# teamtomo/torch-motion-correction

Measured on AMD Instinct MI355X. Metric: frames/sec motion-corrected, 40×4k×4k fp32 stack, 1/2/4/8 MI355X, higher is better.
Workload: dtype f32; 1 GPU; 40-frame 4096x4096 fp32 movie, global rigid shift estimate+correct (estimate_global_motion -> correct_motion, frames + sum out), 1 stack per GPU per step, consecutive steps overlapped on two HIP streams; b_factor=500

## Files before the change

torch_motion_correction_amd/csrc/mc_wave_fft.h:

```cpp
#pragma once

#ifdef __HIPCC__
#include "mc_common.h"
#define MC_HD __host__ __device__ __forceinline__
#else
#include <math.h>
#include <stdint.h>
struct cfloat {
  float x, y;
};
#define MC_HD static inline
#endif

typedef float wf2 __attribute__((ext_vector_type(2)));

#define WF_N 2048
#define WF_SLAB 1024

#ifdef __HIPCC__
__device__ __forceinline__ void wf_sync() {
  __builtin_amdgcn_fence(__ATOMIC_RELEASE, "wavefront");
  __builtin_amdgcn_wave_barrier();
  __builtin_amdgcn_fence(__ATOMIC_ACQUIRE, "wavefront");
}
#endif

MC_HD wf2 wf_make(float re, float im) { return wf2{re, im}; }
MC_HD wf2 wf_from(cfloat c) { return wf2{c.x, c.y}; }
MC_HD cfloat wf_to(wf2 v) { return cfloat{v.x, v.y}; }

MC_HD wf2 wf_add_mi(wf2 a, wf2 b) {
#if defined(__HIP_DEVICE_COMPILE__)
  wf2 r;
  asm("v_pk_add_f32 %0, %1, %2 op_sel:[0,1] op_sel_hi:[1,0] neg_hi:[0,1]" : "=v"(r) : "v"(a), "v"(b));
  return r;
#else
  return wf2{a.x + b.y, a.y - b.x};
#endif
}
MC_HD wf2 wf_sub_mi(wf2 a, wf2 b) {
#if defined(__HIP_DEVICE_COMPILE__)
  wf2 r;
  asm("v_pk_add_f32 %0, %1, %2 op_sel:[0,1] op_sel_hi:[1,0] neg_lo:[0,1]" : "=v"(r) : "v"(a), "v"(b));
  return r;
#else
  return wf2{a.x - b.y, a.y + b.x};
#endif
}
MC_HD wf2 wf_cmul(wf2 a, wf2 w) {
#if defined(__HIP_DEVICE_COMPILE__)
  wf2 t, r;
  asm("v_pk_mul_f32 %0, %1, %2 op_sel_hi:[0,1]" : "=v"(t) : "v"(a), "v"(w));
  asm("v_pk_fma_f32 %0, %1, %2, %3 op_sel:[1,1,0] op_sel_hi:[1,0,1] neg_lo:[0,1,0]"
      : "=v"(r)
      : "v"(a), "v"(w), "v"(t));
  return r;
#else
  return wf2{a.x * w.x - a.y * w.y, a.x * w.y + a.y * w.x};
#endif
}
MC_HD wf2 wf_fma_c(wf2 a, wf2 b, float cr, float ci) {
  const wf2 c = {cr, ci}, cs = {-ci, cr};
  return __builtin_elementwise_fma(b.yy, cs, __builtin_elementwise_fma(b.xx, c, a));
}
MC_HD wf2 wf_cmulc(wf2 a, float cr, float ci) {
  const wf2 c = {cr, ci}, cs = {-ci, cr};
  return __builtin_elementwise_fma(a.yy, cs, a.xx * c);
}

MC_HD void wf_bfly4(wf2& a0, wf2& a1, wf2& a2, wf2& a3) {
  const wf2 t0 = a0 + a2, t1 = a0 - a2;
  const wf2 t2 = a1 + a3, d = a1 - a3;
  a0 = t0 + t2;
  a2 = t0 - t2;
  a1 = wf_add_mi(t1, d);
  a3 = wf_sub_mi(t1, d);
}

MC_HD void wf_dft16(wf2 (&a)[16]) {
  const float C1 = 0.92387953251128673848f, S1 = 0.38268343236508978178f;
  const float H = 0.70710678118654752440f;
#pragma unroll
  for (int j = 0; j < 4; ++j) wf_bfly4(a[j], a[j + 4], a[j + 8], a[j + 12]);
  a[1 + 4] = wf_cmulc(a[1 + 4], C1, -S1);
  a[1 + 8] = wf_cmulc(a[1 + 8], H, -H);
  a[1 + 12] = wf_cmulc(a[1 + 12], S1, -C1);
  a[2 + 4] = wf_cmulc(a[2 + 4], H, -H);
  a[2 + 12] = wf_cmulc(a[2 + 12], -H, -H);
  a[3 + 4] = wf_cmulc(a[3 + 4], S1, -C1);
  a[3 + 8] = wf_cmulc(a[3 + 8], -H, -H);
  a[3 + 12] = wf_cmulc(a[3 + 12], -C1, S1);
#pragma unroll
  for (int p = 0; p < 4; ++p) {
    wf2 &b0 = a[4 * p], &b1 = a[4 * p + 1], &b2 = a[4 * p + 2], &b3 = a[4 * p + 3];
    if (p == 2) {
      const wf2 t0 = wf_add_mi(b0, b2), t1 = wf_sub_mi(b0, b2);
      const wf2 t2 = b1 + b3, d = b1 - b3;
      b0 = t0 + t2;
      b2 = t0 - t2;
      b1 = wf_add_mi(t1, d);
      b3 = wf_sub_mi(t1, d);
    } else {
      wf_bfly4(b0, b1, b2, b3);
    }
  }
#pragma unroll
  for (int p = 0; p < 4; ++p)
#pragma unroll
    for (int r = p + 1; r < 4; ++r) {
      const wf2 s = a[4 * p + r];
      a[4 * p + r] = a[4 * r + p];
      a[4 * r + p] = s;
    }
}

MC_HD void wf_dft16_lo2(wf2 (&a)[16]) {
  const float C1 = 0.92387953251128673848f, S1 = 0.38268343236508978178f;
  const float H = 0.70710678118654752440f;
  const wf2 x0 = a[0], x1 = a[1], x2 = a[14], x3 = a[15];
  a[0] = x0; a[4] = x0; a[8] = x0; a[12] = x0;
  a[1] = x1;
  a[1 + 4] = wf_cmulc(x1, C1, -S1);
  a[1 + 8] = wf_cmulc(x1, H, -H);
  a[1 + 12] = wf_cmulc(x1, S1, -C1);
  a[2] = x2;
  a[2 + 4] = wf_cmulc(x2, H, H);
  a[2 + 8] = -x2;
  a[2 + 12] = wf_cmulc(x2, -H, H);
  a[3] = x3;
  a[3 + 4] = wf_cmulc(x3, C1, S1);
  a[3 + 8] = wf_cmulc(x3, H, H);
  a[3 + 12] = wf_cmulc(x3, S1, C1);
#pragma unroll
  for (int p = 0; p < 4; ++p) {
    wf2 &b0 = a[4 * p], &b1 = a[4 * p + 1], &b2 = a[4 * p + 2], &b3 = a[4 * p + 3];
    if (p == 2) {
      const wf2 t0 = wf_add_mi(b0, b2), t1 = wf_sub_mi(b0, b2);
      const wf2 t2 = b1 + b3, d = b1 - b3;
      b0 = t0 + t2;
      b2 = t0 - t2;
      b1 = wf_add_mi(t1, d);
      b3 = wf_sub_mi(t1, d);
    } else {
      wf_bfly4(b0, b1, b2, b3);
    }
  }
#pragma unroll
  for (int p = 0; p < 4; ++p)
#pragma unroll
    for (int r = p + 1; r < 4; ++r) {
      const wf2 s = a[4 * p + r];
      a[4 * p + r] = a[4 * r + p];
      a[4 * r + p] = s;
    }
}

template <int KEEP>
MC_HD void wf_dft8_pruned(const wf2 (&e)[4], const wf2 (&o)[4], wf2 (&z)[8]) {
  const float H = 0.70710678118654752440f;
  wf2 e0 = e[0], e1 = e[1], e2 = e[2], e3 = e[3];
  wf2 o0 = o[0], o1 = o[1], o2 = o[2], o3 = o[3];
  wf_bfly4(e0, e1, e2, e3);
  wf_bfly4(o0, o1, o2, o3);
  z[0] = e0 + o0;
  z[7] = wf_fma_c(e3, o3, H, H);
  if (KEEP >= 2) {
    z[1] = wf_fma_c(e1, o1, H, -H);
    z[6] = wf_sub_mi(e2, o2);
  }
  if (KEEP >= 4) {
    z[2] = wf_add_mi(e2, o2);
    z[3] = wf_fma_c(e3, o3, -H, -H);
    z[4] = e0 - o0;
    z[5] = wf_fma_c(e1, o1, -H, H);
  }
}

struct WfLane {
  int x1w_base, x1w_mask;
  int x1r[4];
  int x2w;
  int x2r[4];
  int kbin[4];
  int self;
};

MC_HD WfLane wf_lane(int t) {
  WfLane L;
  {
    const int n2 = t >> 2, h1 = (t >> 1) & 1, h0 = t & 1;
    L.x1w_base = (n2 * 2 + h1) * 32 + h0 * 16;
    L.x1w_mask = (n2 & 3) | (h1 << 2) | (h0 << 3);
  }
  {
    const int k1 = t & 15, g2 = t >> 4, h1 = g2 >> 1, h0 = g2 & 1;
    const int lanepart = h1 * 32 + h0 * 16, lo = k1 ^ ((h1 << 2) | (h0 << 3));
    for (int v = 0; v < 4; ++v) L.x1r[v] = lanepart + (lo ^ v);
    L.x2w = g2 * 256 + k1;
  }
  L.kbin[0] = t;
  L.kbin[1] = t == 0 ? 128 : 256 - t;
  L.kbin[2] = 64 + t;
  L.kbin[3] = 192 - t;
  for (int s = 0; s < 4; ++s) L.x2r[s] = L.kbin[s];
  L.self = t == 0;
  return L;
}

MC_HD wf2 wf_unpack(wf2 zk, wf2 zmr, wf2 wk) {
  const wf2 zm = {zmr.x, -zmr.y};
  const wf2 sm = zk + zm, d = zk - zm;
  const wf2 wd = wf_cmul(d, wk);
  return wf_add_mi(sm, wd) * 0.5f;
}

template <int KEEP>
MC_HD void wf_unpack_lane(const wf2 (&z)[4][8], const wf2 (&wk)[4], bool self, wf2 (&X)[4][KEEP]) {
  const float C1 = 0.92387953251128673848f, S1 = 0.38268343236508978178f;
#pragma unroll
  for (int k3 = 0; k3 < KEEP; ++k3) {
    const wf2 m_a0 = self ? z[0][(8 - k3) & 7] : z[1][7 - k3];
    const wf2 m_a1 = self ? z[1][7 - k3] : z[0][7 - k3];
    wf2 w[4] = {wk[0], wk[1], wk[2], wk[3]};
    if (k3 == 1) {
#pragma unroll
      for (int s = 0; s < 4; ++s) w[s] = wf_cmulc(w[s], C1, -S1);
    }
    X[0][k3] = wf_unpack(z[0][k3], m_a0, w[0]);
    X[1][k3] = wf_unpack(z[1][k3], m_a1, w[1]);
    X[2][k3] = wf_unpack(z[2][k3], z[3][7 - k3], w[2]);
    X[3][k3] = wf_unpack(z[3][k3], z[2][7 - k3], w[3]);
  }
}

#define WF5_N 512
#define WF5_SLAB 512

MC_HD void wf_dft8(wf2 (&a)[8]) {
  const float H = 0.70710678118654752440f;
  wf2 e0 = a[0], e1 = a[2], e2 = a[4], e3 = a[6];
  wf2 o0 = a[1], o1 = a[3], o2 = a[5], o3 = a[7];
  wf_bfly4(e0, e1, e2, e3);
  wf_bfly4(o0, o1, o2, o3);
  a[0] = e0 + o0;
  a[4] = e0 - o0;
  a[1] = wf_fma_c(e1, o1, H, -H);
  a[5] = wf_fma_c(e1, o1, -H, H);
  a[2] = wf_add_mi(e2, o2);
  a[6] = wf_sub_mi(e2, o2);
  a[3] = wf_fma_c(e3, o3, -H, -H);
  a[7] = wf_fma_c(e3, o3, H, H);
}

MC_HD int wf5_x1(int k1, int n2, int n3) { return ((n2 * 8 + (k1 ^ n2)) * 8) + (n3 ^ (4 * (k1 >> 2))); }
MC_HD int wf5_x2(int k2, int n3, int k1) { return ((n3 * 8 + (k2 ^ n3)) * 8) + k1; }

#define WF10_N 1024
MC_HD int wf10_x1(int k1, int q) { return k1 * 64 + (q ^ ((2 * k1) & 31)); }
MC_HD int wf10_x2(int k1, int k2, int n3) { return n3 * 128 + k2 * 16 + k1; }

MC_HD void wf_twiddle8(wf2 (&a)[8], wf2 w1) {
  const wf2 w2 = wf_cmul(w1, w1), w3 = wf_cmul(w2, w1), w4 = wf_cmul(w2, w2);
  a[1] = wf_cmul(a[1], w1);
  a[2] = wf_cmul(a[2], w2);
  a[3] = wf_cmul(a[3], w3);
  a[4] = wf_cmul(a[4], w4);
  a[5] = wf_cmul(a[5], wf_cmul(w4, w1));
  a[6] = wf_cmul(a[6], wf_cmul(w4, w2));
  a[7] = wf_cmul(a[7], wf_cmul(w4, w3));
}
MC_HD void wf_twiddle16(wf2 (&a)[16], wf2 w1, wf2 w2, wf2 w4, wf2 w8) {
  const wf2 w3 = wf_cmul(w2, w1), w5 = wf_cmul(w4, w1), w6 = wf_cmul(w4, w2), w7 = wf_cmul(w4, w3);
  a[1] = wf_cmul(a[1], w1); a[2] = wf_cmul(a[2], w2); a[3] = wf_cmul(a[3], w3); a[4] = wf_cmul(a[4], w4);
  a[5] = wf_cmul(a[5], w5); a[6] = wf_cmul(a[6], w6); a[7] = wf_cmul(a[7], w7); a[8] = wf_cmul(a[8], w8);
  a[9] = wf_cmul(a[9], wf_cmul(w8, w1)); a[10] = wf_cmul(a[10], wf_cmul(w8, w2));
  a[11] = wf_cmul(a[11], wf_cmul(w8, w3)); a[12] = wf_cmul(a[12], wf_cmul(w8, w4));
  a[13] = wf_cmul(a[13], wf_cmul(w8, w5)); a[14] = wf_cmul(a[14], wf_cmul(w8, w6));
  a[15] = wf_cmul(a[15], wf_cmul(w8, w7));
}
```

torch_motion_correction_amd/csrc/xc_search.hip:

```cpp
#include "xc_common.h"

__global__ void xc_search_init(int* __restrict__ best, int* __restrict__ gate, float* __restrict__ bounds,
                               int npairs, int nbounds, float* __restrict__ shift_table, int nshift) {
  const int i = blockIdx.x * blockDim.x + threadIdx.x;
  if (i < nbounds) bounds[i] = 0.f;
  if (i < nshift) shift_table[i] = 0.f;
  if (i < npairs) best[i] = (int)0x807fffffu;
  if (i == 0) gate[0] = 0;
}

__global__ void xc_far_needed(const float* __restrict__ bounds, const int* __restrict__ best,
                              float* __restrict__ part_val, int* __restrict__ part_idx,
                              int* __restrict__ need_full, int H, int RG, int near) {
  const int ngrp = H / RG;
  const int p = blockIdx.y;
  const int grp = near + blockIdx.x * blockDim.x + threadIdx.x;
  if (grp >= ngrp - near) return;
  float b = 0.f;
  for (int r = 0; r < RG; ++r) b = fmaxf(b, bounds[(int64_t)p * H + grp * RG + r]);
  b = b * 1.0001f + 1e-30f;
  part_val[(int64_t)p * ngrp + grp] = -INFINITY;
  part_idx[(int64_t)p * ngrp + grp] = 0x7fffffff;
  const int fb = __float_as_int(b);
  if ((fb >= 0 ? fb : fb ^ 0x7fffffff) >= best[p]) atomicOr(need_full, 1);
}



__global__ __launch_bounds__(256) void xc_row_bounds(const cfloat* __restrict__ T2,
                                                     float* __restrict__ bounds, int nkx, int H) {
  __shared__ float part[4][64];
  const int ly = threadIdx.x & 63, slice = threadIdx.x >> 6;
  const int y = blockIdx.x * 64 + ly;
  const int p = blockIdx.y;
  float b0 = 0.f, b1 = 0.f, b2 = 0.f, b3 = 0.f;
  if (y < H) {
    const cfloat* in = T2 + (int64_t)p * nkx * H + y;
    int kx = slice;
    for (; kx + 12 < nkx; kx += 16) {
      const cfloat v0 = in[(int64_t)kx * H], v1 = in[(int64_t)(kx + 4) * H];
      const cfloat v2 = in[(int64_t)(kx + 8) * H], v3 = in[(int64_t)(kx + 12) * H];
      b0 += (kx == 0 ? 1.f : 2.f) * sqrtf(v0.x * v0.x + v0.y * v0.y);
      b1 += 2.f * sqrtf(v1.x * v1.x + v1.y * v1.y);
      b2 += 2.f * sqrtf(v2.x * v2.x + v2.y * v2.y);
      b3 += 2.f * sqrtf(v3.x * v3.x + v3.y * v3.y);
    }
    for (; kx < nkx; kx += 4) {
      const cfloat v = in[(int64_t)kx * H];
      b0 += (kx == 0 ? 1.f : 2.f) * sqrtf(v.x * v.x + v.y * v.y);
    }
  }
  part[slice][ly] = (b0 + b1) + (b2 + b3);
  __syncthreads();
  if (slice == 0 && y < H)
    bounds[(int64_t)p * H + y] = (part[0][ly] + part[1][ly]) + (part[2][ly] + part[3][ly]);
}

template <int LOGN, int EPI>
__global__ __launch_bounds__(MC_WG) void xc_rows_inv(const cfloat* __restrict__ T2,
                                                     const float* __restrict__ bounds,
                                                     int* __restrict__ best,
                                                     float* __restrict__ part_val,
                                                     int* __restrict__ part_idx,
                                                     float* __restrict__ out_real,
                                                     const int64_t* __restrict__ out_off,
                                                     int64_t out_stride,
                                                     const cfloat* __restrict__ tw_row, XcGeom g,
                                                     int near, int phase, int compact,
                                                     const int* __restrict__ gate) {
  constexpr int N = 1 << LOGN;
  if (gate && gate[0] == 0) return;
  constexpr int NT = fft_threads(N), SG = MC_WG / NT;
  constexpr int R0 = FftPlan<N>::radix(0), NB0 = N / R0, IT0 = (NB0 + NT - 1) / NT;
  extern __shared__ __attribute__((aligned(16))) char smem[];
  const int tid = threadIdx.x;
  const int lt = tid & (NT - 1), sg = tid / NT;
  cfloat* l0 = reinterpret_cast<cfloat*>(smem) + sg * 2 * lds_len(N);
  cfloat* l1 = l0 + lds_len(N);
  cfloat* stg = reinterpret_cast<cfloat*>(smem) + SG * 2 * lds_len(N);
  const int p = blockIdx.y;
  const int RG = g.RG;
  const int ngrp = g.H / RG;
  int grp = blockIdx.x;
  if (EPI == 0) grp = phase == 0 ? ((int)blockIdx.x < near ? (int)blockIdx.x : ngrp - 2 * near + (int)blockIdx.x)
                                 : near + (int)blockIdx.x;
  if constexpr (EPI == 0) {
    if (phase == 1) {
      float b = 0.f;
      for (int r = 0; r < RG; ++r) b = fmaxf(b, bounds[(int64_t)p * g.H + grp * RG + r]);
      b = b * 1.0001f + 1e-30f;
      if (float_order(b) < __hip_atomic_load(&best[p], __ATOMIC_RELAXED, __HIP_MEMORY_SCOPE_AGENT)) {
        if (tid == 0) {
          part_val[(int64_t)p * ngrp + grp] = -INFINITY;
          part_idx[(int64_t)p * ngrp + grp] = 0x7fffffff;
        }
        return;
      }
    }
  }
  const int nstore = near * RG + (compact > 0 ? compact - 1 : 0);
  const int cstride = compact ? 2 * nstore : g.H;
  const int coff = (int)blockIdx.x < near ? (int)blockIdx.x * RG
                                          : nstore + (compact - 1) + ((int)blockIdx.x - near) * RG;
  const cfloat* in = T2 + (int64_t)p * g.nkx * cstride + (int64_t)(compact ? coff : grp * RG);
  for (int i0 = tid; i0 < g.nkx * RG; i0 += 8 * MC_WG) {
    cfloat v8[8];
#pragma unroll
    for (int u = 0; u < 8; ++u) {
      const int i = i0 + u * MC_WG;
      const int kx = i / RG, r = i - kx * RG;
      if (i < g.nkx * RG) v8[u] = in[(int64_t)kx * cstride + r];
    }
#pragma unroll
    for (int u = 0; u < 8; ++u) {
      const int i = i0 + u * MC_WG;
      const int kx = i / RG, r = i - kx * RG;
      if (i < g.nkx * RG) stg[kx * (RG + 1) + r] = v8[u];
    }
  }
  FftTwiddles<N> T;
  T.template init<+1>(lt, tw_row, 2);
  cfloat wk[IT0][R0];
#pragma unroll
  for (int it = 0; it < IT0; ++it)
#pragma unroll
    for (int q = 0; q < R0; ++q) {
      const int j = lt + it * NT;
      const int k = (NB0 % NT == 0 || j < NB0) ? j + q * NB0 : 0;
      cfloat w = tw_row[k];
      w.y = -w.y;
      wk[it][q] = w;
    }
  __syncthreads();
  float bv = -INFINITY;
  int bi = 0x7fffffff;
  int s = 0;
  for (int r = sg; r < RG; r += SG) {
    const int y = grp * RG + r;
    auto load = [&](int k, int it, int q) {
      const int km = N - k;
      cfloat xk = (k < g.nkx) ? stg[k * (RG + 1) + r] : cmake(0.f, 0.f);
      cfloat xm = (km < g.nkx) ? cconj(stg[km * (RG + 1) + r]) : cmake(0.f, 0.f);
      if (k == 0) {
        xk.y = 0.f;
        xm.y = 0.f;
      }
      const cfloat sm = cadd(xk, xm), d = csub(xk, xm);
      const cfloat wd = cmul(wk[it][q], d);
      return cmake(sm.x - wd.y, sm.y + wd.x);
    };
    int res;
    if constexpr (EPI == 0) {
      auto store = [&](int n, cfloat v) {
        const int flat = y * g.W + 2 * n;
        cand_merge(bv, bi, v.x, flat);
        cand_merge(bv, bi, v.y, flat + 1);
      };
      res = wg_fft_pp<N, +1, true>(l0, l1, s, lt, T, load, store);
    } else {
      float* orow = out_real + out_off[p] + (int64_t)y * out_stride;
      auto store = [&](int n, cfloat v) {
        orow[2 * n] = v.x;
        orow[2 * n + 1] = v.y;
      };
      res = wg_fft_pp<N, +1, true>(l0, l1, s, lt, T, load, store);
    }
    s = res ^ 1;
  }
  if constexpr (EPI == 0) {
    for (int off = 32; off > 0; off >>= 1) {
      const float ov = __shfl_down(bv, off);
      const int oi = __shfl_down(bi, off);
      cand_merge(bv, bi, ov, oi);
    }
    __shared__ float wv[MC_WG / 64];
    __shared__ int wi[MC_WG / 64];
    if ((tid & 63) == 0) {
      wv[tid >> 6] = bv;
      wi[tid >> 6] = bi;
    }
    __syncthreads();
    if (tid == 0) {
      for (int w = 1; w < MC_WG / 64; ++w) cand_merge(bv, bi, wv[w], wi[w]);
      part_val[(int64_t)p * ngrp + grp] = bv;
      part_idx[(int64_t)p * ngrp + grp] = bi;
      atomicMax(&best[p], float_order(bv));
    }
  }
}

__global__ void xc_peak_final(const float* __restrict__ part_val, const int* __restrict__ part_idx,
                              int ngrp, int H, int W, int* __restrict__ peaks,
                              float* __restrict__ shifts, const int* __restrict__ shift_rows) {
  const int p = blockIdx.x;
  float bv = -INFINITY;
  int bi = 0x7fffffff;
  for (int i = threadIdx.x; i < ngrp; i += blockDim.x)
    cand_merge(bv, bi, part_val[(int64_t)p * ngrp + i], part_idx[(int64_t)p * ngrp + i]);
  for (int off = 32; off > 0; off >>= 1) {
    const float ov = __shfl_down(bv, off);
    const int oi = __shfl_down(bi, off);
    cand_merge(bv, bi, ov, oi);
  }
  if (threadIdx.x == 0) {
    if (bi == 0x7fffffff) bi = 0;
    peaks[p] = bi;
    const int py = bi / W, px = bi - py * W;
    const int row = shift_rows ? shift_rows[p] : p;
    shifts[2 * row] = (float)(py <= H / 2 ? py : py - H);
    shifts[2 * row + 1] = (float)(px <= W / 2 ? px : px - W);
  }
}

template <int LOGN>
__global__ __launch_bounds__(MC_WG) void xc_peak_nbhd(const cfloat* __restrict__ T2,
                                                      const int* __restrict__ peaks,
                                                      float* __restrict__ nb,
                                                      const cfloat* __restrict__ tw_row, XcGeom g,
                                                      const cfloat* __restrict__ T2n,
                                                      const int* __restrict__ gate, int nstore) {
  constexpr int N = 1 << LOGN;
  __shared__ __attribute__((aligned(16))) cfloat line[lds_len(N)];
  const int tid = threadIdx.x;
  const int p = blockIdx.y, dy = (int)blockIdx.x - 1;
  const int pk = peaks[p];
  const int py = pk / g.W, px = pk - py * g.W;
  const int y = py + dy;
  float* o = nb + (int64_t)p * 9 + (dy + 1) * 3;
  if (y < 0 || y >= g.H) {
    if (tid < 3) o[tid] = __builtin_nanf("");
    return;
  }
  const cfloat* in = T2 + (int64_t)p * g.nkx * g.H + y;
  int64_t cs = g.H;
  if (T2n && gate[0] == 0) {
    const int yn = y < nstore ? y : y - (g.H - 2 * nstore);
    if (yn < 0 || yn >= 2 * nstore || (y >= nstore && y < g.H - nstore)) {
      if (tid < 3) o[tid] = __builtin_nanf("");
      return;
    }
    cs = 2 * nstore;
    in = T2n + (int64_t)p * g.nkx * cs + yn;
  }
  auto X = [&](int k) { return in[(int64_t)k * cs]; };
  auto load = [&](int k) {
    const int km = N - k;
    cfloat xk = (k < g.nkx) ? X(k) : cmake(0.f, 0.f);
    cfloat xm = (km < g.nkx) ? cconj(X(km)) : cmake(0.f, 0.f);
    if (k == 0) {
      xk.y = 0.f;
      xm.y = 0.f;
    }
    const cfloat s = cadd(xk, xm), d = csub(xk, xm);
    cfloat w = tw_row[k];
    w.y = -w.y;
    const cfloat wd = cmul(w, d);
    return cmake(s.x - wd.y, s.y + wd.x);
  };
  auto store = [&](int n, cfloat v) { line[lpad(n)] = v; };
  wg_fft<N, +1>(line, tid, tw_row, 2, load, store);
  __syncthreads();
  if (tid < 3) {
    const int x = px + tid - 1;
    float v = __builtin_nanf("");
    if (x >= 0 && x < g.W) {
      const cfloat z = line[lpad(x >> 1)];
      v = (x & 1) ? z.y : z.x;
    }
    o[tid] = v;
  }
}

void mc_launch_row_bounds(const cfloat* T2, float* bounds, int nkx, int H, int npairs, hipStream_t stream) {
  hipLaunchKernelGGL(xc_row_bounds, dim3((H + 63) / 64, npairs), dim3(256), 0, stream, T2, bounds, nkx, H);
}
void mc_launch_peak_final(const float* part_val, const int* part_idx, int ngrp, int H, int W, int* peaks,
                          float* shifts, const int* shift_rows, int npairs, hipStream_t stream) {
  hipLaunchKernelGGL(xc_peak_final, dim3(npairs), dim3(64), 0, stream, part_val, part_idx, ngrp, H, W, peaks, shifts,
                     shift_rows);
}

constexpr int XC_NEAR_GUARD = 8;

using RowsInvKernel = decltype(&xc_rows_inv<4, 0>);
template <int EPI>
static int rows_inv_kernel(const XcGeom& g, RowsInvKernel* k, size_t* lds) {
  *lds = rows_lds_bytes(g.W / 2, g);
  MC_DISPATCH_LOG(mc_ilog2(g.W) - 1, *k = xc_rows_inv<L, EPI>);
  return mc_dyn_lds(*k, *lds);
}
static void rows_argmax_launch(RowsInvKernel k, size_t lds, int ngroups, int npairs, const void* T2, const float* bounds,
                               int* best, float* part_val, int* part_idx, const void* tw_row, const XcGeom& g,
                               int near, int phase, int compact, const int* gate, hipStream_t stream) {
  hipLaunchKernelGGL(k, dim3(ngroups, npairs), dim3(MC_WG), lds, stream, (const cfloat*)T2, bounds, best, part_val,
                     part_idx, (float*)nullptr, (const int64_t*)nullptr, (int64_t)0, (const cfloat*)tw_row, g, near,
                     phase, compact, gate);
}

extern "C" {

int mc_xc_rows_inverse_argmax(const void* T2, float* part_val, int* part_idx, int* peaks,
                              float* shifts, const void* tw_row, int npairs, const mc_xc_geom* q,
                              void* stream) {
  XcGeom g;
  int rc = geom_from(q, &g, true, false);
  if (rc) return rc;
  if (!T2 || !part_val || !part_idx || !peaks || !shifts || !tw_row || npairs < 1)
    return MC_ERR_ARG;
  hipStream_t st = (hipStream_t)stream;
  RowsInvKernel k;
  size_t lds;
  if ((rc = rows_inv_kernel<0>(g, &k, &lds))) return rc;
  const int ngrp = g.H / g.RG;
  int* best = part_idx + (int64_t)npairs * ngrp;
  {
    const float ninf = -INFINITY;
    int pat;
    memcpy(&pat, &ninf, 4);
    pat = pat >= 0 ? pat : pat ^ 0x7fffffff;
    hipError_t e = hipMemsetD32Async((hipDeviceptr_t)best, pat, npairs, st);
    if (e != hipSuccess) return (int)e;
  }
  const int near = xc_near_groups(g), nfar = ngrp - 2 * near;
  float* bounds = part_val + (int64_t)npairs * ngrp;
  if (nfar > 0) mc_launch_row_bounds((const cfloat*)T2, bounds, g.nkx, g.H, npairs, st);
  if (near > 0)
    rows_argmax_launch(k, lds, 2 * near, npairs, T2, bounds, best, part_val, part_idx, tw_row, g, near, 0, 0, nullptr, st);
  if (nfar > 0)
    rows_argmax_launch(k, lds, nfar, npairs, T2, bounds, best, part_val, part_idx, tw_row, g, near, 1, 0, nullptr, st);
  rc = mc_check_launch();
  if (rc) return rc;
  mc_launch_peak_final(part_val, part_idx, ngrp, g.H, g.W, peaks, shifts, nullptr, npairs, st);
  return mc_check_launch();
}

int mc_xc_near_rows(const mc_xc_geom* q) {
  XcGeom g;
  int rc = geom_from(q, &g, true, true);
  if (rc) return rc;
  return xc_near_groups(g) * g.RG + XC_NEAR_GUARD;
}

int mc_xc_correlate_argmax(const void* S_cur, const int* cur_idx, const void* S_ref,
                           const int* ref_idx, void* T2_full, void* T2_near, float* part_val,
                           int* part_idx, int* peaks, float* shifts, const int* shift_rows,
                           int n_shift_rows, float* nb, const void* tw_col, const void* tw_row,
                           float scale, int npairs, const mc_xc_geom* q, void* stream) {
  XcGeom g;
  int rc = geom_from(q, &g, true, true);
  if (rc) return rc;
  if (!S_cur || !cur_idx || !S_ref || !ref_idx || !T2_full || !T2_near || !part_val || !part_idx ||
      !peaks || !shifts || !tw_col || !tw_row || npairs < 1)
    return MC_ERR_ARG;
  if (g.H < 1024) return MC_ERR_UNSUPPORTED;
  hipStream_t st = (hipStream_t)stream;
  RowsInvKernel k;
  size_t lds;
  if ((rc = rows_inv_kernel<0>(g, &k, &lds))) return rc;
  const int ngrp = g.H / g.RG;
  const int near = xc_near_groups(g);
  if (near < 1) return MC_ERR_UNSUPPORTED;
  const int nstore = near * g.RG + XC_NEAR_GUARD;
  if (nstore > 256) return MC_ERR_UNSUPPORTED;
  int* best = part_idx + (int64_t)npairs * ngrp;
  int* gate = best + npairs;
  float* bounds = part_val + (int64_t)npairs * ngrp;
  if (shift_rows && n_shift_rows < 1) return MC_ERR_ARG;
  hipLaunchKernelGGL(xc_search_init, dim3((npairs * g.H + 255) / 256), dim3(256), 0, st, best, gate, bounds,
                     npairs, npairs * g.H, shifts, shift_rows ? 2 * n_shift_rows : 0);
  rc = mc_launch_cols_inv_near((const cfloat*)S_cur, cur_idx, (const cfloat*)S_ref, ref_idx, (cfloat*)T2_near, bounds,
                               (const cfloat*)tw_col, scale, g, nstore, npairs, st);
  if (rc) return rc;
  rows_argmax_launch(k, lds, 2 * near, npairs, T2_near, bounds, best, part_val, part_idx, tw_row, g, near, 0,
                     1 + XC_NEAR_GUARD, nullptr, st);
  rc = mc_check_launch();
  if (rc) return rc;
  const int nfar = ngrp - 2 * near;
  if (nfar > 0) {
    hipLaunchKernelGGL(xc_far_needed, dim3((nfar + 63) / 64, npairs), dim3(64), 0, st,
                       (const float*)bounds, (const int*)best, part_val, part_idx, gate, g.H, g.RG, near);
    rc = mc_launch_cols_inv_gated((const cfloat*)S_cur, cur_idx, (const cfloat*)S_ref, ref_idx, (cfloat*)T2_full,
                                  (const cfloat*)tw_col, scale, g, gate, npairs, st);
    if (rc) return rc;
    rows_argmax_launch(k, lds, nfar, npairs, T2_full, bounds, best, part_val, part_idx, tw_row, g, near, 1, 0, gate, st);
    rc = mc_check_launch();
    if (rc) return rc;
  }
  mc_launch_peak_final(part_val, part_idx, ngrp, g.H, g.W, peaks, shifts, shift_rows, npairs, st);
  if (nb) {
    MC_DISPATCH_LOG(mc_ilog2(g.W) - 1, {
      hipLaunchKernelGGL(xc_peak_nbhd<L>, dim3(3, npairs), dim3(MC_WG), 0, st, (const cfloat*)T2_full,
                         (const int*)peaks, nb, (const cfloat*)tw_row, g, (const cfloat*)T2_near,
                         (const int*)gate, nstore);
    });
  }
  return mc_check_launch();
}

int mc_xc_rows_inverse_store(const void* T2, float* out, const int64_t* out_off,
                             int64_t out_stride, const void* tw_row, int nframes,
                             const mc_xc_geom* q, void* stream) {
  XcGeom g;
  int rc = geom_from(q, &g, true, false);
  if (rc) return rc;
  if (!T2 || !out || !out_off || !tw_row || nframes < 1) return MC_ERR_ARG;
  RowsInvKernel k;
  size_t lds;
  if ((rc = rows_inv_kernel<1>(g, &k, &lds))) return rc;
  hipLaunchKernelGGL(k, dim3(g.H / g.RG, nframes), dim3(MC_WG), lds, (hipStream_t)stream, (const cfloat*)T2,
                     (const float*)nullptr, (int*)nullptr, (float*)nullptr, (int*)nullptr, out, out_off, out_stride,
                     (const cfloat*)tw_row, g, 0, 0, 0, (const int*)nullptr);
  return mc_check_launch();
}

int mc_xc_peak_neighbourhood(const void* T2, const int* peaks, float* nb, const void* tw_row,
                             int npairs, const mc_xc_geom* q, void* stream) {
  XcGeom g;
  int rc = geom_from(q, &g, true, false);
  if (rc) return rc;
  if (!T2 || !peaks || !nb || !tw_row || npairs < 1) return MC_ERR_ARG;
  const int logn = mc_ilog2(g.W) - 1;
  dim3 grid(3, npairs);
  MC_DISPATCH_LOG(logn, {
    hipLaunchKernelGGL(xc_peak_nbhd<L>, grid, dim3(MC_WG), 0, (hipStream_t)stream,
                       (const cfloat*)T2, peaks, nb, (const cfloat*)tw_row, g, (const cfloat*)nullptr,
                       (const int*)nullptr, 0);
  });
  return mc_check_launch();
}

}
```

Before: 24680 frames/s.

## Add wavefront-local pruned inverse row FFT with fused argmax for xcorr search

Adds a new row-inverse kernel that runs a 4096-point real inverse FFT per wavefront using register-level radix-16 stages, pruned inputs (only the low kx bins live, KEEP=1/2), and fused running argmax, with twiddles cached in LDS. It replaces the generic rows_inv kernel on the cross-correlation search path when W=4096 and nkx<=512. The aim is to cut LDS traffic, block-level syncs and wasted butterflies on zero-padded bins in the peak search. It adds substantial hand-written FFT code whose correctness depends on intricate index and packing logic.

Result: no change. 24870 frames/s, median of 6 (+0.8%).

```diff
diff --git a/torch_motion_correction_amd/csrc/mc_wave_fft.h b/torch_motion_correction_amd/csrc/mc_wave_fft.h
--- a/torch_motion_correction_amd/csrc/mc_wave_fft.h
+++ b/torch_motion_correction_amd/csrc/mc_wave_fft.h
@@ -233,6 +233,91 @@
   }
 }
 
+
+MC_HD wf2 wf_cmul_conj(wf2 a, wf2 w) {
+#if defined(__HIP_DEVICE_COMPILE__)
+  wf2 t, r;
+  asm("v_pk_mul_f32 %0, %1, %2 op_sel_hi:[0,1] neg_hi:[0,1]" : "=v"(t) : "v"(a), "v"(w));
+  asm("v_pk_fma_f32 %0, %1, %2, %3 op_sel:[1,1,0] op_sel_hi:[1,0,1]" : "=v"(r) : "v"(a), "v"(w), "v"(t));
+  return r;
+#else
+  return wf2{a.x * w.x + a.y * w.y, a.y * w.x - a.x * w.y};
+#endif
+}
+MC_HD wf2 wf_conj(wf2 a) { return wf2{a.x, -a.y}; }
+
+MC_HD void wf_idft16(wf2 (&a)[16]) {
+  wf_dft16(a);
+#pragma unroll
+  for (int j = 1; j < 8; ++j) {
+    const wf2 s = a[j];
+    a[j] = a[16 - j];
+    a[16 - j] = s;
+  }
+}
+
+template <int KEEP, int PAR>
+MC_HD void wf_idft8_live(const wf2 (&z)[8], wf2 (&b)[4]) {
+  const float H = 0.70710678118654752440f;
+  const wf2 hh = {H, H};
+  if (KEEP == 1) {
+    if (PAR == 0) {
+      b[0] = z[0] + z[7];
+      b[1] = wf_add_mi(z[0], z[7]);
+      b[2] = z[0] - z[7];
+      b[3] = wf_sub_mi(z[0], z[7]);
+    } else {
+      b[0] = wf_fma_c(z[0], z[7], H, -H);
+      b[1] = wf_fma_c(z[0], z[7], -H, -H);
+      b[2] = wf_fma_c(z[0], z[7], -H, H);
+      b[3] = wf_fma_c(z[0], z[7], H, H);
+    }
+  } else {
+    const wf2 p = z[1] + z[7], m = z[1] - z[7];
+    if (PAR == 0) {
+      const wf2 e0 = z[0] + z[6], e2 = z[0] - z[6];
+      b[0] = e0 + p;
+      b[1] = wf_sub_mi(e2, m);
+      b[2] = e0 - p;
+      b[3] = wf_add_mi(e2, m);
+    } else {
+      const wf2 e1 = wf_add_mi(z[0], z[6]), e3 = wf_sub_mi(z[0], z[6]);
+      const wf2 u = wf_sub_mi(p, m), v = wf_add_mi(p, m);
+      b[0] = __builtin_elementwise_fma(u, hh, e1);
+      b[1] = __builtin_elementwise_fma(v, -hh, e3);
+      b[2] = __builtin_elementwise_fma(u, -hh, e1);
+      b[3] = __builtin_elementwise_fma(v, hh, e3);
+    }
+  }
+}
+
+template <int KEEP>
+MC_HD void wf_pack_lane(const wf2 (&X)[4][KEEP], const wf2 (&wk)[4], bool self, wf2 (&z)[4][8]) {
+  const float C1 = 0.92387953251128673848f, S1 = 0.38268343236508978178f;
+  wf2 zm[4][KEEP];
+#pragma unroll
+  for (int s = 0; s < 4; ++s)
+#pragma unroll
+    for (int k3 = 0; k3 < KEEP; ++k3) {
+      wf2 x = X[s][k3];
+      if (s == 0 && k3 == 0) x.y = self ? 0.f : x.y;
+      const wf2 w = k3 == 1 ? wf_cmulc(wk[s], C1, -S1) : wk[s];
+      const wf2 wd = wf_cmul_conj(x, w);
+      z[s][k3] = wf_sub_mi(x, wd);
+      zm[s][k3] = wf_conj(wf_add_mi(x, wd));
+    }
+  const wf2 zero = {0.f, 0.f};
+#pragma unroll
+  for (int k3 = 0; k3 < KEEP; ++k3) {
+    z[1][7 - k3] = self ? zm[1][k3] : zm[0][k3];
+    z[0][7 - k3] = self ? (k3 + 1 < KEEP ? zm[0][k3 + 1 < KEEP ? k3 + 1 : 0] : zero) : zm[1][k3];
+    z[3][7 - k3] = zm[2][k3];
+    z[2][7 - k3] = zm[3][k3];
+  }
+}
+
+MC_HD int wf_inv_x(int t, int h, int n1, int j) { return 256 * n1 + 4 * t + 2 * h + j; }
+
 #define WF5_N 512
 #define WF5_SLAB 512
 
diff --git a/torch_motion_correction_amd/csrc/xc_search.hip b/torch_motion_correction_amd/csrc/xc_search.hip
--- a/torch_motion_correction_amd/csrc/xc_search.hip
+++ b/torch_motion_correction_amd/csrc/xc_search.hip
@@ -1,4 +1,5 @@
 #include "xc_common.h"
+#include "mc_wave_fft.h"
 
 __global__ void xc_search_init(int* __restrict__ best, int* __restrict__ gate, float* __restrict__ bounds,
                                int npairs, int nbounds, float* __restrict__ shift_table, int nshift) {
@@ -189,6 +190,205 @@
   }
 }
 
+#define WF_TWA (4 * 128)
+#define WF_TWB (4 * 15 * 2)
+
+__device__ __forceinline__ void wi_pin(int& v, float dep) { asm volatile("" : "+v"(v) : "v"(dep)); }
+
+template <int KEEP, int H>
+__device__ __forceinline__ void wf_inv_half(const wf2 (&X)[4][KEEP], int t, wf2* slab, const cfloat* twA,
+                                            const cfloat* twB, const cfloat* twK, int flat0, float& bv, int& bi) {
+  wi_pin(t, H ? bv : X[0][0].x);
+  const WfLane L = wf_lane(t);
+  wf2 a[16];
+#pragma unroll
+  for (int pr = 0; pr < 4; pr += 2) {
+    wf2 z[4][8], b[2][4], wk[4];
+#pragma unroll
+    for (int s = 0; s < 4; ++s) wk[s] = wf_from(twK[64 * s + t]);
+    wf_pack_lane<KEEP>(X, wk, L.self != 0, z);
+#pragma unroll
+    for (int s = 0; s < 2; ++s) wf_idft8_live<KEEP, H>(z[pr + s], b[s]);
+#pragma unroll
+    for (int s = 0; s < 2; ++s)
+#pragma unroll
+      for (int n3h = 0; n3h < 4; ++n3h) slab[L.x2r[pr + s] + 256 * n3h] = b[s][n3h];
+    __builtin_amdgcn_sched_barrier(0);
+  }
+  wf_sync();
+#pragma unroll
+  for (int k2 = 0; k2 < 16; ++k2) a[k2] = slab[L.x2w + 16 * k2];
+  wf_sync();
+  wi_pin(t, a[15].y);
+  const WfLane L1 = wf_lane(t);
+  {
+    const cfloat* twb = twB + (t >> 4) * 30 + H;
+#pragma unroll
+    for (int k2 = 1; k2 < 16; ++k2) a[k2] = wf_cmul_conj(a[k2], wf_from(twb[2 * (k2 - 1)]));
+  }
+  wf_idft16(a);
+#pragma unroll
+  for (int n2 = 0; n2 < 16; ++n2) slab[L1.x1r[n2 & 3] + 64 * n2] = a[n2];
+  wf_sync();
+#pragma unroll
+  for (int k1 = 0; k1 < 16; ++k1) a[k1] = slab[L1.x1w_base + (k1 ^ L1.x1w_mask)];
+  wf_sync();
+  wi_pin(t, a[15].y);
+  {
+    const cfloat* twa = twA + 2 * t + H;
+    wf_twiddle16(a, wf_conj(wf_from(twa[0])), wf_conj(wf_from(twa[128])), wf_conj(wf_from(twa[256])),
+                 wf_conj(wf_from(twa[384])));
+  }
+  wf_idft16(a);
+  const bool first = (a[0].x > bv) | ((a[0].x == bv) & (flat0 + 4 * t < bi));
+  bv = first ? a[0].x : bv;
+  int code = first ? 0 : -1;
+#pragma unroll
+  for (int n1 = 0; n1 < 16; ++n1) {
+    const int off = wf_inv_x(0, 0, n1, 0);
+    if (n1 > 0) {
+      const bool gx = a[n1].x > bv;
+      bv = gx ? a[n1].x : bv;
+      code = gx ? off : code;
+    }
+    const bool gy = a[n1].y > bv;
+    bv = gy ? a[n1].y : bv;
+    code = gy ? off + 1 : code;
+  }
+  bi = code >= 0 ? flat0 + 4 * t + code : bi;
+}
+
+template <int KEEP>
+__global__ __launch_bounds__(256, 4) void xc_rows_inv_wave(const cfloat* __restrict__ T2,
+                                                           const float* __restrict__ bounds,
+                                                           int* __restrict__ best, float* __restrict__ part_val,
+                                                           int* __restrict__ part_idx,
+                                                           const cfloat* __restrict__ tw_row, XcGeom g, int near,
+                                                           int phase, int compact, const int* __restrict__ gate) {
+  constexpr int RR = 8, RPW = RR / 4;
+  constexpr int SWS = 2;
+  if (gate && gate[0] == 0) return;
+  __shared__ __attribute__((aligned(16))) cfloat slabs[4][WF_SLAB];
+  __shared__ __attribute__((aligned(16))) cfloat tab[WF_TWA + WF_TWB + 256];
+  const cfloat* twA = tab;
+  const cfloat* twB = tab + WF_TWA;
+  const cfloat* twK = tab + WF_TWA + WF_TWB;
+  const int tid = threadIdx.x, t = tid & 63;
+  const int wv = __builtin_amdgcn_readfirstlane(tid >> 6);
+  const int p = blockIdx.y;
+  const int RG = g.RG;
+  const int ngrp = g.H / RG;
+  const int grp = phase == 0 ? ((int)blockIdx.x < near ? (int)blockIdx.x : ngrp - 2 * near + (int)blockIdx.x)
+                             : near + (int)blockIdx.x;
+  if (phase == 1) {
+    float b = 0.f;
+    for (int r = 0; r < RG; ++r) b = fmaxf(b, bounds[(int64_t)p * g.H + grp * RG + r]);
+    b = b * 1.0001f + 1e-30f;
+    if (float_order(b) < __hip_atomic_load(&best[p], __ATOMIC_RELAXED, __HIP_MEMORY_SCOPE_AGENT)) {
+      if (tid == 0) {
+        part_val[(int64_t)p * ngrp + grp] = -INFINITY;
+        part_idx[(int64_t)p * ngrp + grp] = 0x7fffffff;
+      }
+      return;
+    }
+  }
+  {
+    constexpr int NTAB = WF_TWA + WF_TWB + 256, PER = (NTAB + 255) / 256;
+    cfloat tv[PER];
+#pragma unroll
+    for (int j = 0; j < PER; ++j) {
+      int i = tid + 256 * j;
+      i = i < NTAB ? i : NTAB - 1;
+      int src_k;
+      if (i < WF_TWA) {
+        src_k = (2 * (i & 127)) << (i >> 7);
+      } else if (i < WF_TWA + WF_TWB) {
+        const int e = i - WF_TWA, h = e & 1, k2 = ((e >> 1) % 15) + 1, gq = e / 30;
+        src_k = 32 * (2 * gq + h) * k2;
+      } else {
+        const int e = i - WF_TWA - WF_TWB, sl = e >> 6, l = e & 63;
+        src_k = sl == 0 ? l : (sl == 1 ? (l == 0 ? 128 : 256 - l) : (sl == 2 ? 64 + l : 192 - l));
+      }
+      tv[j] = tw_row[src_k];
+    }
+#pragma unroll
+    for (int j = 0; j < PER; ++j) {
+      const int i = tid + 256 * j;
+      if (i < NTAB) tab[i] = tv[j];
+    }
+  }
+  const int nstore = near * RG + (compact > 0 ? compact - 1 : 0);
+  const int cstride = compact ? 2 * nstore : g.H;
+  const int coff = (int)blockIdx.x < near ? (int)blockIdx.x * RG
+                                          : nstore + (compact - 1) + ((int)blockIdx.x - near) * RG;
+  const cfloat* in = T2 + (int64_t)p * g.nkx * cstride + (int64_t)(compact ? coff : grp * RG);
+  cfloat* stage = &slabs[0][0];
+  wf2* slab = reinterpret_cast<wf2*>(slabs[wv]);
+  float bv = -INFINITY, bv1 = -INFINITY;
+  int bi = 0x7fffffff, bi1 = 0x7fffffff;
+#pragma unroll 1
+  for (int r0 = 0; r0 < RG; r0 += RR) {
+    if (r0) __syncthreads();
+    int ts = threadIdx.x;
+    wi_pin(ts, bv);
+    const int tl = ts & 63;
+    for (int i0 = ts; i0 < g.nkx * RR; i0 += 8 * 256) {
+      cfloat v8[8];
+#pragma unroll
+      for (int u = 0; u < 8; ++u) {
+        const int i = i0 + u * 256;
+        const int kx = i / RR, r = i & (RR - 1);
+        if (i < g.nkx * RR) v8[u] = in[(int64_t)kx * cstride + r0 + r];
+      }
+#pragma unroll
+      for (int u = 0; u < 8; ++u) {
+        const int i = i0 + u * 256;
+        const int kx = i / RR, r = i & (RR - 1);
+        if (i < g.nkx * RR) stage[kx * RR + (r ^ ((kx >> SWS) & (RR - 1)))] = v8[u];
+      }
+    }
+    __syncthreads();
+    wf2 X[RPW][4][KEEP];
+    const WfLane L = wf_lane(tl);
+#pragma unroll
+    for (int j = 0; j < RPW; ++j)
+#pragma unroll
+      for (int s = 0; s < 4; ++s)
+#pragma unroll
+        for (int k3 = 0; k3 < KEEP; ++k3) {
+          const int k = L.kbin[s] + 256 * k3, r = 4 * j + wv;
+          const cfloat v = stage[k * RR + (r ^ ((k >> SWS) & (RR - 1)))];
+          X[j][s][k3] = k < g.nkx ? wf_from(v) : wf2{0.f, 0.f};
+        }
+    __syncthreads();
+#pragma unroll
+    for (int j = 0; j < RPW; ++j) {
+      const int flat0 = (grp * RG + r0 + 4 * j + wv) * g.W;
+      wf_inv_half<KEEP, 0>(X[j], tl, slab, twA, twB, twK, flat0, bv, bi);
+      wf_inv_half<KEEP, 1>(X[j], tl, slab, twA, twB, twK, flat0 + 2, bv1, bi1);
+    }
+  }
+  cand_merge(bv, bi, bv1, bi1);
+  for (int off = 32; off > 0; off >>= 1) {
+    const float ov = __shfl_down(bv, off);
+    const int oi = __shfl_down(bi, off);
+    cand_merge(bv, bi, ov, oi);
+  }
+  __shared__ float wvv[4];
+  __shared__ int wvi[4];
+  if (t == 0) {
+    wvv[wv] = bv;
+    wvi[wv] = bi;
+  }
+  __syncthreads();
+  if (tid == 0) {
+    for (int w = 1; w < 4; ++w) cand_merge(bv, bi, wvv[w], wvi[w]);
+    part_val[(int64_t)p * ngrp + grp] = bv;
+    part_idx[(int64_t)p * ngrp + grp] = bi;
+    atomicMax(&best[p], float_order(bv));
+  }
+}
+
 __global__ void xc_peak_final(const float* __restrict__ part_val, const int* __restrict__ part_idx,
                               int ngrp, int H, int W, int* __restrict__ peaks,
                               float* __restrict__ shifts, const int* __restrict__ shift_rows) {
@@ -289,9 +489,21 @@
   MC_DISPATCH_LOG(mc_ilog2(g.W) - 1, *k = xc_rows_inv<L, EPI>);
   return mc_dyn_lds(*k, *lds);
 }
-static void rows_argmax_launch(RowsInvKernel k, size_t lds, int ngroups, int npairs, const void* T2, const float* bounds,
-                               int* best, float* part_val, int* part_idx, const void* tw_row, const XcGeom& g,
-                               int near, int phase, int compact, const int* gate, hipStream_t stream) {
+static int rows_wave_keep(const XcGeom& g) {
+  if (g.W != 4096 || g.nkx > 512) return 0;
+  const int keep = g.nkx <= 256 ? 1 : 2;
+  return g.RG % 8 ? 0 : keep;
+}
+static void rows_argmax_launch(RowsInvKernel k, size_t lds, int wave_keep, int ngroups, int npairs, const void* T2,
+                               const float* bounds, int* best, float* part_val, int* part_idx, const void* tw_row,
+                               const XcGeom& g, int near, int phase, int compact, const int* gate,
+                               hipStream_t stream) {
+  if (wave_keep) {
+    auto kw = wave_keep == 1 ? xc_rows_inv_wave<1> : xc_rows_inv_wave<2>;
+    hipLaunchKernelGGL(kw, dim3(ngroups, npairs), dim3(256), 0, stream, (const cfloat*)T2, bounds, best, part_val,
+                       part_idx, (const cfloat*)tw_row, g, near, phase, compact, gate);
+    return;
+  }
   hipLaunchKernelGGL(k, dim3(ngroups, npairs), dim3(MC_WG), lds, stream, (const cfloat*)T2, bounds, best, part_val,
                      part_idx, (float*)nullptr, (const int64_t*)nullptr, (int64_t)0, (const cfloat*)tw_row, g, near,
                      phase, compact, gate);
@@ -325,9 +537,9 @@
   float* bounds = part_val + (int64_t)npairs * ngrp;
   if (nfar > 0) mc_launch_row_bounds((const cfloat*)T2, bounds, g.nkx, g.H, npairs, st);
   if (near > 0)
-    rows_argmax_launch(k, lds, 2 * near, npairs, T2, bounds, best, part_val, part_idx, tw_row, g, near, 0, 0, nullptr, st);
+    rows_argmax_launch(k, lds, 0, 2 * near, npairs, T2, bounds, best, part_val, part_idx, tw_row, g, near, 0, 0, nullptr, st);
   if (nfar > 0)
-    rows_argmax_launch(k, lds, nfar, npairs, T2, bounds, best, part_val, part_idx, tw_row, g, near, 1, 0, nullptr, st);
+    rows_argmax_launch(k, lds, 0, nfar, npairs, T2, bounds, best, part_val, part_idx, tw_row, g, near, 1, 0, nullptr, st);
   rc = mc_check_launch();
   if (rc) return rc;
   mc_launch_peak_final(part_val, part_idx, ngrp, g.H, g.W, peaks, shifts, nullptr, npairs, st);
@@ -357,6 +569,7 @@
   RowsInvKernel k;
   size_t lds;
   if ((rc = rows_inv_kernel<0>(g, &k, &lds))) return rc;
+  const int wave = rows_wave_keep(g);
   const int ngrp = g.H / g.RG;
   const int near = xc_near_groups(g);
   if (near < 1) return MC_ERR_UNSUPPORTED;
@@ -371,7 +584,7 @@
   rc = mc_launch_cols_inv_near((const cfloat*)S_cur, cur_idx, (const cfloat*)S_ref, ref_idx, (cfloat*)T2_near, bounds,
                                (const cfloat*)tw_col, scale, g, nstore, npairs, st);
   if (rc) return rc;
-  rows_argmax_launch(k, lds, 2 * near, npairs, T2_near, bounds, best, part_val, part_idx, tw_row, g, near, 0,
+  rows_argmax_launch(k, lds, wave, 2 * near, npairs, T2_near, bounds, best, part_val, part_idx, tw_row, g, near, 0,
                      1 + XC_NEAR_GUARD, nullptr, st);
   rc = mc_check_launch();
   if (rc) return rc;
@@ -382,7 +595,7 @@
     rc = mc_launch_cols_inv_gated((const cfloat*)S_cur, cur_idx, (const cfloat*)S_ref, ref_idx, (cfloat*)T2_full,
                                   (const cfloat*)tw_col, scale, g, gate, npairs, st);
     if (rc) return rc;
-    rows_argmax_launch(k, lds, nfar, npairs, T2_full, bounds, best, part_val, part_idx, tw_row, g, near, 1, 0, gate, st);
+    rows_argmax_launch(k, lds, wave, nfar, npairs, T2_full, bounds, best, part_val, part_idx, tw_row, g, near, 1, 0, gate, st);
     rc = mc_check_launch();
     if (rc) return rc;
   }
```
